# DylanAuty/ObjCAViT

Measured on AMD Instinct MI355X. Metric: images/sec (640x480, bs=16) forward depth inference, 3 batches of 16 in flight per GPU; AbsRel vs CPU ref, higher is better.
Workload: dtype f32 (fp16 / bf16 split contractions)

## Files before the change

### include/objcavit_hip.h

```cpp
#ifndef OBJCAVIT_HIP_H
#define OBJCAVIT_HIP_H

#include <stddef.h>
#include <stdint.h>

#ifdef __cplusplus
extern "C" {
#endif

typedef void* ocv_stream_t;

#define OCV_ABI_VERSION 5
int ocv_abi_version(void);
const char* ocv_last_error(void);

int ocv_range_flag_set(unsigned* flag);
int ocv_range_flag_take_fwd(unsigned* flag, unsigned* out, ocv_stream_t stream);
int ocv_attention_set_fp32_range(int on);
int ocv_attention_set_dispatch(int form);

#define OCV_ACT_NONE 0
#define OCV_ACT_RELU 1
#define OCV_ACT_LEAKY_RELU 2
#define OCV_ACT_SILU 3
// ... 126 lines not shown
int ocv_pointwise_conv_nhwc_split_fwd(const float* x, const float* gate, int rows_per_image, const void* w_packed,
                                      const float* bias, const float* residual, float* y, long M, int Cin, int Cout,
                                      int act, ocv_stream_t stream);
int ocv_pointwise_conv_nhwc_split_hl_fwd(const float* x, const float* gate, int rows_per_image, const void* w_packed,
                                         const float* bias, const float* residual, float* y, void* y_hl, long M, int Cin,
                                         int Cout, int act, ocv_stream_t stream);
size_t ocv_pointwise_split_workspace_bytes(long M, int Cin, int Cout);
int ocv_pointwise_conv_nhwc_split_ws_fwd(const float* x, const float* gate, int rows_per_image, const void* w_packed,
                                         const float* bias, const float* residual, float* y, void* y_hl, long M, int Cin, int Cout,
                                         int act, void* workspace, size_t workspace_bytes, ocv_stream_t stream);
int ocv_pointwise_hl_set_dispatch(int rt, int tn);
int ocv_pointwise_hl_fwd(const void* x_hl, int Cin, const void* w_packed, long w_image_elems, int rows_per_image,
                         const float* bias, const float* residual, float* y, void* y_hl, long M, int Cout, int act,
                         ocv_stream_t stream);
int ocv_stem_conv_fwd(const float* x, const float* w, const float* bias, float* y, int B, int Cin, int H, int W, int Cout,
                      int k, int stride, int pad_t, int pad_l, int Ho, int Wo, int act, ocv_stream_t stream);
int ocv_depthwise_conv_nhwc_fwd(const float* in, const float* w, const float* bias, float* out, int B, int C, int H,
                                int W, int k, int stride, int pad_t, int pad_l, int Ho, int Wo, int act,
                                ocv_stream_t stream);
int ocv_depthwise_set_dispatch(int mode);
int ocv_depthwise_sum_tiles(int B, int C, int Ho, int Wo, int k, int stride);
int ocv_depthwise_conv_nhwc_sum_fwd(const float* in, const float* w, const float* bias, float* out, float* part, int B,
                                    int C, int H, int W, int k, int stride, int pad_t, int pad_l, int Ho, int Wo,
                                    ocv_stream_t stream);
int ocv_se_gate_partials_fwd(const float* part, int tiles, long pixels_per_image, const float* w1, const float* b1,
                             const float* w2t, const float* b2, float* gate, float* hidden_ws, int B, int C, int R,
                             ocv_stream_t stream);
int ocv_depthwise_conv_nhwc_sum_hl_fwd(const float* in, const float* w, const float* bias, float* out, void* out_hl, float* part,
                                       int B, int C, int H, int W, int k, int stride, int pad_t, int pad_l, int Ho, int Wo,
                                       ocv_stream_t stream);
int ocv_se_gate_weights_fwd(const float* part, int tiles, long pixels_per_image, const float* w1, const float* b1,
                            const float* w2t, const float* b2, const float* W, void* w_packed, long w_image_elems, float* gate,
                            float* hidden_ws, int B, int C, int R, int N, ocv_stream_t stream);


size_t ocv_channel_mean_workspace_bytes(int B, int C, long P);
int ocv_channel_mean_nhwc_fwd(const float* x, float* out, int B, int C, long P, void* workspace, size_t workspace_bytes,
                              ocv_stream_t stream);

int ocv_se_gate_fwd(const float* mean, const float* w1, const float* b1, const float* w2t, const float* b2, float* gate,
                    float* hidden_ws, int B, int C, int R, ocv_stream_t stream);

int ocv_conv_nhwc_fwd(const float* x1, int C1, const float* x2, int C2, const void* w_hi, const void* w_lo,
                      const float* bias, const float* residual, float* y, int B, int H, int W, int Cout, int ksize,
                      int act, ocv_stream_t stream);
int ocv_conv_nhwc_exact_fwd(const float* x1, int C1, const float* x2, int C2, const float* w_tap_major, const float* bias,
                            const float* residual, float* y, int B, int H, int W, int Cout, int ksize, int act,
                            ocv_stream_t stream);
int ocv_conv3x3_nhwc_strided_fwd(const float* x, int Cin, const void* w_hi, const void* w_lo, const float* bias,
                                 const float* residual, float* y, int B, int H, int W, int Cout, int stride, int pad_t,
                                 int pad_l, int Ho, int Wo, int act, ocv_stream_t stream);

int ocv_mbconv_expand_dw_tiles(int Ho, int Wo, int k, int stride);
int ocv_mbconv_expand_dw_fwd(const float* x, const void* w_packed, const float* bias_expand, const float* w_dw,
                             const float* bias_dw, float* y, float* part, int B, int H, int W, int Cin, int mid, int k,
                             int stride, int pad_t, int pad_l, int Ho, int Wo, ocv_stream_t stream);

size_t ocv_split_act_elems(int B, int H, int W, int C);

int ocv_conv_nhwc_split_fwd(const void* x_hl, int Cin, const void* w_hi, const void* w_lo, const float* bias,
                            const float* residual, float* y, void* y_hl, int B, int H, int W, int Cout, int ksize,
                            int act, ocv_stream_t stream);
size_t ocv_conv_nhwc_split_workspace_bytes(int B, int H, int W, int Cin, int Cout, int ksize);
int ocv_conv_nhwc_split_ws_fwd(const void* x_hl, int Cin, const void* w_hi, const void* w_lo, const float* bias,
                               const float* residual, float* y, void* y_hl, int B, int H, int W, int Cout, int ksize,
                               int act, void* workspace, size_t workspace_bytes, ocv_stream_t stream);
int ocv_conv_nhwc_split_x_fwd(const void* x_hl, int Cin, const void* w_hi, const void* w_lo, const float* oscale, int f16,
                              const float* bias, const float* residual, float* y, void* y_hl, int B, int H, int W, int Cout,
                              int ksize, int act, void* workspace, size_t workspace_bytes, ocv_stream_t stream);

int ocv_conv3x3_packed_taps_k(int Cin);
int ocv_conv3x3_halo_supported(int B, int H, int W, int Cin, int Cout);
size_t ocv_conv3x3_halo_lds_bytes(void);
int ocv_conv3x3_set_dispatch(int mode);
int ocv_conv3x3_last_kernel(void);
int ocv_conv3x3_split_packed_taps_fwd(const void* x_hl, int Cin, const void* w_hi, const void* w_lo, const float* oscale, int f16,
                                      const float* bias, const float* residual, float* y, void* y_hl, int B, int H, int W, int Cout,
                                      int act, ocv_stream_t stream);

size_t ocv_conv3x3_winograd43_workspace_bytes(int B, int H, int W, int Cin, int Cout);
int ocv_conv3x3_winograd43_split_fwd(const void* x_hl, int Cin, const void* u_hi, const void* u_lo, const float* fscale,
                                     const float* cscale, const float* bias, float* y, void* y_hl, int B, int H, int W, int Cout,
                                     int act, int hl_f16, void* workspace, size_t workspace_bytes, ocv_stream_t stream);

int ocv_tap_interp_supported(int h, int w, int H, int W, int Cout);
int ocv_tap_interp_staging_rounds(int h, int w, int H, int W);
int ocv_tap_interp_combine_fwd(const float* z, int h, int w, int zpad, const float* zborder, const float* s, const float* bias,
                               float* y, void* y_hl, int B, int H, int W, int Cout, int act, ocv_stream_t stream);
int ocv_tap_interp_combine_x_fwd(const float* z, int h, int w, int zpad, const float* zborder, const float* s, const float* bias,
                                 float* y, void* y_hl, int hl_f16, int B, int H, int W, int Cout, int act, ocv_stream_t stream);


int ocv_upsample_concat_split_fwd(const float* x, int h, int w, int C1, const float* skip, int C2, void* out_hl, int B,
                                  int H, int W, ocv_stream_t stream);
int ocv_upsample_concat_split_x_fwd(const float* x, int h, int w, int C1, const float* skip, int C2, void* out_hl, int f16, int B,
                                    int H, int W, ocv_stream_t stream);

size_t ocv_depth_metrics_workspace_bytes(int B, int H, int W);
int ocv_depth_metrics_fwd(const float* pred, const float* pred_mirror, int h, int w, const float* gt, int H, int W,
                          float min_depth, float max_depth, int crop_y0, int crop_y1, int crop_x0, int crop_x1,
                          long first_image_id, float* records, int B, void* workspace, size_t workspace_bytes,
                          ocv_stream_t stream);
size_t ocv_depth_metrics_loss_workspace_bytes(int B, int H, int W, int n_bins);
int ocv_depth_metrics_loss_fwd(const float* pred, const float* pred_mirror, int h, int w, const float* gt, int H, int W,
                               float min_depth, float max_depth, int crop_y0, int crop_y1, int crop_x0, int crop_x1,
                               const float* bin_edges, int n_bins, long first_image_id, float* records, float* loss_records, int B,
// ... 65 lines not shown
```

### objcavit_amd/_lib.py

```python
from __future__ import annotations

import ctypes as C
import os
from typing import Optional

_HERE = os.path.dirname(os.path.abspath(__file__))
LIB_PATH = os.environ.get("OCV_LIB_PATH") or os.path.join(_HERE, "lib", "libobjcavit_hip.so")

_f32p = C.c_void_p
_u8p = C.c_void_p
_stream = C.c_void_p
ABI_VERSION = 5


class EncoderLayerParams(C.Structure):
    _fields_ = [("struct_size", C.c_size_t)] + [(n, C.c_void_p) for n in (
        "in_proj_w", "in_proj_b", "out_proj_w", "out_proj_b", "norm1_w", "norm1_b",
        "linear1_w", "linear1_b", "linear2_w", "linear2_b", "norm2_w", "norm2_b",
        "in_proj_p3", "out_proj_p3", "linear1_p3", "linear2_p3",
        "in_proj_h2", "out_proj_h2", "linear1_h2", "linear2_h2")]

    def __init__(self, *a, **kw):
        super().__init__(*a, **kw)
        self.struct_size = C.sizeof(EncoderLayerParams)
# ... 71 lines not shown
    "ocv_bin_head_partials_bytes": (C.c_size_t, [C.c_int, C.c_int]),
    "ocv_bin_head_folded_ws_fwd": (C.c_int, [_f32p, C.c_int, _f32p, _f32p, _f32p, _f32p, C.c_int, C.c_int, C.c_int, C.c_int,
                                             C.c_void_p, C.c_size_t, _stream]),
    "ocv_bin_head_stats_partials_bytes": (C.c_size_t, [C.c_int, C.c_int]),
    "ocv_bin_head_folded_stats_fwd": (C.c_int, [_f32p, C.c_int, _f32p, _f32p, _f32p, _f32p, C.c_int, C.c_int, C.c_int, C.c_int,
                                                C.c_void_p, C.c_size_t, _f32p, _f32p, _stream]),
    "ocv_bin_head_fwd": (C.c_int, [_f32p, C.c_int, _f32p, C.c_long, C.c_int, _f32p, _f32p, _f32p, _f32p, C.c_int, C.c_int,
                                   C.c_int, C.c_int, C.c_int, C.c_void_p, C.c_size_t, _stream]),
    "ocv_depthwise_conv_fwd": (C.c_int, [_f32p, _f32p, _f32p, _f32p] + [C.c_int] * 11 + [_stream]),
    "ocv_depthwise_set_dispatch": (C.c_int, [C.c_int]),
    "ocv_depthwise_sum_tiles": (C.c_int, [C.c_int] * 6),
    "ocv_depthwise_conv_nhwc_sum_fwd": (C.c_int, [_f32p] * 5 + [C.c_int] * 10 + [_stream]),
    "ocv_se_gate_partials_fwd": (C.c_int, [_f32p, C.c_int, C.c_long, _f32p, _f32p, _f32p, _f32p, _f32p, _f32p, C.c_int,
                                           C.c_int, C.c_int, _stream]),
    "ocv_depth_metrics_workspace_bytes": (C.c_size_t, [C.c_int] * 3),
    "ocv_depth_metrics_fwd": (C.c_int, [_f32p, _f32p, C.c_int, C.c_int, _f32p, C.c_int, C.c_int, C.c_float, C.c_float] + [C.c_int] * 4 +
                              [C.c_long, _f32p, C.c_int, C.c_void_p, C.c_size_t, _stream]),
    "ocv_depth_metrics_loss_workspace_bytes": (C.c_size_t, [C.c_int] * 4),
    "ocv_depth_metrics_loss_fwd": (C.c_int, [_f32p, _f32p, C.c_int, C.c_int, _f32p, C.c_int, C.c_int, C.c_float, C.c_float] + [C.c_int] * 4 +
                                   [_f32p, C.c_int, C.c_long, _f32p, _f32p, C.c_int, C.c_void_p, C.c_size_t, _stream]),
    "ocv_frame_ingest_fwd": (C.c_int, [_u8p, C.c_long, C.c_long, C.c_int, C.c_int, C.c_int, C.c_int, _f32p, _f32p, C.c_int, C.c_int, C.c_int,
                                       C.c_int, C.c_long, _stream]),
    "ocv_depth_ingest_fwd": (C.c_int, [C.c_void_p, C.c_long, C.c_long, C.c_int, C.c_int, C.c_int, C.c_int, C.c_float, _f32p, C.c_int, C.c_int,
                                       C.c_int, _stream]),
    "ocv_depth_finalize_fwd": (C.c_int, [_f32p, _f32p, C.c_int, C.c_int, C.c_float, C.c_float, C.c_int, C.c_int, _f32p, C.c_void_p, C.c_float,
                                         _u8p, _u8p, C.c_float, C.c_float, C.c_int, _stream]),
    "ocv_depth_finalize_stats_fwd": (C.c_int, [_f32p] * 6 + [C.c_int, C.c_int, C.c_float, C.c_float, C.c_int, C.c_int, _f32p, _f32p, C.c_int,
                                               _stream]),
    "ocv_object_depth_fwd": (C.c_int, [_f32p, _f32p, _f32p, C.c_long, C.c_void_p, C.c_int, C.c_int, C.c_int, C.c_int, C.c_float,
                                       C.POINTER(C.c_double), C.c_int, _f32p, _stream]),
    "ocv_object_metrics_workspace_bytes": (C.c_size_t, [C.c_int] * 3),
    "ocv_object_metrics_fwd": (C.c_int, [_f32p, _f32p, C.c_int, C.c_int, _f32p, C.c_int, C.c_int, C.c_float, C.c_float] + [C.c_int] * 4 +
                               [_f32p, C.c_long, C.c_void_p, C.c_int, C.c_int, C.c_float, _f32p, _f32p, C.c_void_p, C.c_size_t, _stream]),
    "ocv_depth_unproject_workspace_bytes": (C.c_size_t, [C.c_int] * 5),
    "ocv_depth_unproject_fwd": (C.c_int, [_f32p, _f32p, _f32p, _f32p, _u8p, C.c_long, C.c_long] + [C.c_int] * 9 + [C.c_float] * 4 +
                                [C.c_int, _f32p, C.c_void_p, C.c_void_p, C.c_void_p, C.c_void_p, C.c_size_t, _stream]),
    "ocv_conv3x3_few_channels_fwd": (C.c_int, [_f32p, C.c_long, C.c_long, C.c_long, C.c_long, _f32p, _f32p] + [C.c_int] * 5 + [_stream]),
    "ocv_stem_conv_fwd": (C.c_int, [_f32p, _f32p, _f32p, _f32p] + [C.c_int] * 12 + [_stream]),
    "ocv_pointwise_packed_weight_elems": (C.c_size_t, [C.c_int, C.c_int]),
    "ocv_pointwise_split_set_dispatch": (C.c_int, [C.c_int, C.c_int, C.c_int]),
    "ocv_pointwise_conv_nhwc_split_fwd": (C.c_int, [_f32p, _f32p, C.c_int, C.c_void_p, _f32p, _f32p, _f32p,
                                                    C.c_long, C.c_int, C.c_int, C.c_int, C.c_void_p]),
    "ocv_pointwise_conv_nhwc_fwd": (C.c_int, [_f32p, _f32p, C.c_int, _f32p, _f32p, _f32p, _f32p, C.c_long, C.c_int, C.c_int,
                                              C.c_int, _stream]),
    "ocv_depthwise_conv_nhwc_fwd": (C.c_int, [_f32p, _f32p, _f32p, _f32p] + [C.c_int] * 11 + [_stream]),
    "ocv_channel_mean_workspace_bytes": (C.c_size_t, [C.c_int, C.c_int, C.c_long]),
    "ocv_channel_mean_nhwc_fwd": (C.c_int, [_f32p, _f32p, C.c_int, C.c_int, C.c_long, C.c_void_p, C.c_size_t, _stream]),
    "ocv_se_gate_fwd": (C.c_int, [_f32p] * 7 + [C.c_int] * 3 + [_stream]),
    "ocv_conv_nhwc_fwd": (C.c_int, [_f32p, C.c_int, _f32p, C.c_int, C.c_void_p, C.c_void_p, _f32p, _f32p, _f32p] +
                          [C.c_int] * 6 + [_stream]),
    "ocv_conv3x3_nhwc_strided_fwd": (C.c_int, [_f32p, C.c_int, C.c_void_p, C.c_void_p, _f32p, _f32p, _f32p] + [C.c_int] * 10 + [_stream]),
    "ocv_conv_nhwc_exact_fwd": (C.c_int, [_f32p, C.c_int, _f32p, C.c_int, _f32p, _f32p, _f32p, _f32p] + [C.c_int] * 6 + [_stream]),
    "ocv_mbconv_expand_dw_tiles": (C.c_int, [C.c_int] * 4),
    "ocv_mbconv_expand_dw_fwd": (C.c_int, [_f32p, C.c_void_p, _f32p, _f32p, _f32p, _f32p, _f32p] + [C.c_int] * 11 + [_stream]),
    "ocv_regressor_bins_fwd": (C.c_int, [_f32p, C.c_long, _f32p, _f32p, _f32p, _f32p, _f32p, _f32p, C.c_int, C.c_int, C.c_int, C.c_int, C.c_float,
                                         C.c_int, C.c_float, C.c_float, _f32p, _f32p, _f32p, C.c_int, _stream]),
    "ocv_bin_edges_fwd": (C.c_int, [_f32p, C.c_int, C.c_float, C.c_float, _f32p, _f32p, _f32p, C.c_int, C.c_int, _stream]),
    "ocv_object_tokens_pad_fwd": (C.c_int, [_f32p, C.c_void_p, C.c_float, _f32p, _u8p, C.c_int, C.c_int, C.c_int, _stream]),
    "ocv_object_front_pad_fwd": (C.c_int, [_f32p, C.c_void_p, C.c_int, C.c_int, C.c_float, _f32p, _u8p] + [C.c_int] * 4 + [_stream]),
    "ocv_object_frontend_fwd": (C.c_int, [_f32p, C.c_long, C.c_void_p, C.c_void_p, C.c_int, C.c_int, C.c_void_p, C.c_int, C.c_void_p, C.c_void_p,
                                          C.c_int, C.c_void_p, C.c_int, C.POINTER(C.c_float), C.c_int, C.c_int, C.c_float, _f32p, C.c_long,
                                          C.c_long, _f32p, C.c_long, C.c_long, C.c_void_p, C.c_int, C.c_void_p, C.c_void_p, _u8p, _stream]),
    "ocv_split_act_elems": (C.c_size_t, [C.c_int] * 4),
    "ocv_conv_nhwc_split_fwd": (C.c_int, [C.c_void_p, C.c_int, C.c_void_p, C.c_void_p, _f32p, _f32p, _f32p, C.c_void_p]
                                + [C.c_int] * 6 + [_stream]),
    "ocv_conv_nhwc_split_workspace_bytes": (C.c_size_t, [C.c_int] * 6),
    "ocv_conv_nhwc_split_ws_fwd": (C.c_int, [C.c_void_p, C.c_int, C.c_void_p, C.c_void_p, _f32p, _f32p, _f32p, C.c_void_p]
                                   + [C.c_int] * 6 + [C.c_void_p, C.c_size_t, _stream]),
    "ocv_conv_nhwc_split_x_fwd": (C.c_int, [C.c_void_p, C.c_int, C.c_void_p, C.c_void_p, _f32p, C.c_int, _f32p, _f32p, _f32p, C.c_void_p]
                                  + [C.c_int] * 6 + [C.c_void_p, C.c_size_t, _stream]),
    "ocv_conv3x3_packed_taps_k": (C.c_int, [C.c_int]),
    "ocv_conv3x3_halo_supported": (C.c_int, [C.c_int] * 5),
    "ocv_conv3x3_halo_lds_bytes": (C.c_size_t, []),
    "ocv_conv3x3_set_dispatch": (C.c_int, [C.c_int]),
    "ocv_conv3x3_last_kernel": (C.c_int, []),
    "ocv_conv3x3_split_packed_taps_fwd": (C.c_int, [C.c_void_p, C.c_int, C.c_void_p, C.c_void_p, _f32p, C.c_int, _f32p, _f32p, _f32p, C.c_void_p]
                                          + [C.c_int] * 5 + [_stream]),
    "ocv_upsample_concat_split_x_fwd": (C.c_int, [_f32p, C.c_int, C.c_int, C.c_int, _f32p, C.c_int, C.c_void_p, C.c_int,
                                                  C.c_int, C.c_int, C.c_int, _stream]),
    "ocv_tap_interp_combine_x_fwd": (C.c_int, [_f32p, C.c_int, C.c_int, C.c_int, _f32p, _f32p, _f32p, _f32p, C.c_void_p] + [C.c_int] * 6 + [_stream]),
    "ocv_pos_grid_sample_fwd": (C.c_int, [_f32p, C.c_int, C.c_int, C.c_int, _f32p, C.c_int, C.c_int, C.c_int, C.c_float, C.c_float,
                                          C.c_int, _f32p, _f32p, _stream]),
    "ocv_conv3x3_winograd43_workspace_bytes": (C.c_size_t, [C.c_int] * 5),
    "ocv_conv3x3_winograd43_split_fwd": (C.c_int, [C.c_void_p, C.c_int, C.c_void_p, C.c_void_p, _f32p, _f32p, _f32p, _f32p, C.c_void_p] + [C.c_int] * 6 +
                                         [C.c_void_p, C.c_size_t, _stream]),
    "ocv_tap_interp_supported": (C.c_int, [C.c_int] * 5),
    "ocv_tap_interp_staging_rounds": (C.c_int, [C.c_int] * 4),
    "ocv_tap_interp_combine_fwd": (C.c_int, [_f32p, C.c_int, C.c_int, C.c_int, _f32p, _f32p, _f32p, _f32p, C.c_void_p] + [C.c_int] * 5 + [_stream]),
    "ocv_upsample_concat_split_fwd": (C.c_int, [_f32p, C.c_int, C.c_int, C.c_int, _f32p, C.c_int, C.c_void_p,
                                                C.c_int, C.c_int, C.c_int, _stream]),
}

_lib: Optional[C.CDLL] = None


class HipLibraryError(RuntimeError):
    pass


def load(path: Optional[str] = None) -> C.CDLL:
    global _lib
    if _lib is not None and path is None:
        return _lib
    import torch
    p = path or LIB_PATH
    if not os.path.exists(p):
# ... 26 lines not shown
```

### objcavit_amd/csrc/mbconv_fused.hip

```cpp
#include "common.hpp"
#include "../../include/objcavit_hip.h"

namespace {

typedef __bf16 bf16x8 __attribute__((ext_vector_type(8)));

struct FXArgs {
  const float *x, *be, *wd, *bd;
  const __bf16* wp;
  float *y, *part;
  int Cin, mid, H, W, Ho, Wo, pad_t, pad_l;
  int tiles_x, tiles_per_image, nchunks;
};

template <int K, int S>
struct FXGeom {
  static constexpr int TH = 8, TW = S == 1 ? 32 : 16;
  static constexpr int RG = 256 / (8 * TW);
  static constexpr int NR = TH / RG;
  static constexpr int IH = (TH - 1) * S + K, IW = (TW - 1) * S + K;
  static constexpr int P = IH * IW, MT = (P + 31) / 32;
  static constexpr int HALF = (IW + 1) / 2;
  static constexpr int NLI = (NR - 1) * S + K;
  static constexpr int LDS_BYTES = MT * 32 * 32 * 4;
// ... 135 lines not shown
      const int d = li - ky;
      if (d >= 0 && d % S == 0 && d / S < G::NR) {
#pragma unroll
        for (int kx = 0; kx < K; ++kx) acc[d / S] = fx_fma4(wdw[ky * K + kx], v[kx], acc[d / S]);
      }
    }
  }
  float4 psum = make_float4(0.f, 0.f, 0.f, 0.f);
  const int ox = ox0 + col;
  float* orow = p.y + (((long)b * p.Ho + oy0 + rg * G::NR) * p.Wo + ox) * p.mid + cq;
  const long ostep = (long)p.Wo * p.mid;
#pragma unroll
  for (int o = 0; o < G::NR; ++o, orow += ostep) {
    const int oy = oy0 + rg * G::NR + o;
    if (cok && oy < p.Ho && ox < p.Wo) {
      float4 r = acc[o];
      r.x = fast_silu(r.x); r.y = fast_silu(r.y); r.z = fast_silu(r.z); r.w = fast_silu(r.w);
      *reinterpret_cast<float4*>(orow) = r;
      psum.x += r.x; psum.y += r.y; psum.z += r.z; psum.w += r.w;
    }
  }
  __syncthreads();
  *reinterpret_cast<float4*>(e + (tid >> 3) * 32 + 4 * q) = psum;
  __syncthreads();
  if (tid < 32 && n0 + tid < p.mid) {
    float s = 0.f;
#pragma unroll 8
    for (int j = 0; j < 32; ++j) s += e[j * 32 + tid];
    p.part[((long)b * p.tiles_per_image + t2) * p.mid + n0 + tid] = s;
  }
}

template <int K, int S, int KS>
int fx_launch(const FXArgs& a, int B, hipStream_t st) {
  using G = FXGeom<K, S>;
  static bool attr = false;
  if (!attr) {
    (void)hipFuncSetAttribute((const void*)mbconv_expand_dw_kernel<K, S, KS>, hipFuncAttributeMaxDynamicSharedMemorySize, G::LDS_BYTES);
    attr = true;
  }
  const long grid = (long)B * a.tiles_per_image * a.nchunks;
  hipLaunchKernelGGL((mbconv_expand_dw_kernel<K, S, KS>), dim3((unsigned)grid), dim3(256), G::LDS_BYTES, st, a);
  OCV_CHECK_LAUNCH("ocv_mbconv_expand_dw_fwd");
  return 0;
}

template <int K, int S>
int fx_dispatch_ks(const FXArgs& a, int B, int ks, hipStream_t st) {
  if (ks == 2) return fx_launch<K, S, 2>(a, B, st);
  if (ks == 3) return fx_launch<K, S, 3>(a, B, st);
  return fx_launch<K, S, 4>(a, B, st);
}

}

extern "C" int ocv_mbconv_expand_dw_tiles(int Ho, int Wo, int k, int stride) {
  if (Ho < 1 || Wo < 1 || (k != 3 && k != 5) || (stride != 1 && stride != 2)) return 0;
  const int tw = stride == 1 ? 32 : 16;
  return ((Ho + 7) / 8) * ((Wo + tw - 1) / tw);
}

namespace {
int fx_run(const float* x, const void* w_packed, const float* bias_expand, const float* w_dw, const float* bias_dw, float* y,
           float* part, int B, int H, int W, int Cin, int mid, int k, int stride, int pad_t, int pad_l,
           int Ho, int Wo, ocv_stream_t stream) {
  OCV_CHECK_ARG(x && w_packed && w_dw && y && part, "ocv_mbconv_expand_dw_fwd: null pointer");
  OCV_CHECK_ARG(B >= 1 && H >= 1 && W >= 1 && Ho >= 1 && Wo >= 1, "ocv_mbconv_expand_dw_fwd: bad sizes");
  OCV_CHECK_ARG(Cin >= 24 && Cin % 8 == 0 && Cin <= 64, "ocv_mbconv_expand_dw_fwd: Cin must be a multiple of 8 in [24, 64] (got %d)", Cin);
  OCV_CHECK_ARG(mid >= 4 && mid % 4 == 0, "ocv_mbconv_expand_dw_fwd: expanded channels must be a multiple of 4 (got %d)", mid);
  OCV_CHECK_ARG((k == 3 || k == 5) && (stride == 1 || stride == 2), "ocv_mbconv_expand_dw_fwd: k must be 3 or 5 and stride 1 or 2 (got k=%d s=%d)", k, stride);
  OCV_CHECK_ARG(pad_t >= 0 && pad_l >= 0 && pad_t < k && pad_l < k, "ocv_mbconv_expand_dw_fwd: bad padding");
  OCV_CHECK_ARG((Ho - 1) * stride - pad_t < H && (Wo - 1) * stride - pad_l < W, "ocv_mbconv_expand_dw_fwd: output larger than the padded input allows");
  OCV_CHECK_ARG(ocv_aligned16(x) && ocv_aligned16(w_packed) && ocv_aligned16(w_dw) && ocv_aligned16(bias_dw) && ocv_aligned16(y),
                "ocv_mbconv_expand_dw_fwd: operands must be 16-byte aligned");
  FXArgs a{};
  a.x = x; a.be = bias_expand; a.wd = w_dw; a.bd = bias_dw; a.wp = (const __bf16*)w_packed; a.y = y; a.part = part;
  a.Cin = Cin; a.mid = mid; a.H = H; a.W = W; a.Ho = Ho; a.Wo = Wo; a.pad_t = pad_t; a.pad_l = pad_l;
  const int tw = stride == 1 ? 32 : 16;
  a.tiles_x = (Wo + tw - 1) / tw;
  a.tiles_per_image = ((Ho + 7) / 8) * a.tiles_x;
  a.nchunks = (mid + 31) / 32;
  OCV_CHECK_ARG((long)B * a.tiles_per_image * a.nchunks < (1L << 31), "ocv_mbconv_expand_dw_fwd: too many work items");
  const int ks = (Cin + 15) / 16;
  hipStream_t st = (hipStream_t)stream;
  if (k == 3 && stride == 1) return fx_dispatch_ks<3, 1>(a, B, ks, st);
  if (k == 3 && stride == 2) return fx_dispatch_ks<3, 2>(a, B, ks, st);
  if (k == 5 && stride == 1) return fx_dispatch_ks<5, 1>(a, B, ks, st);
  return fx_dispatch_ks<5, 2>(a, B, ks, st);
}
}

extern "C" int ocv_mbconv_expand_dw_fwd(const float* x, const void* w_packed, const float* bias_expand, const float* w_dw,
                                        const float* bias_dw, float* y, float* part, int B, int H, int W, int Cin, int mid,
                                        int k, int stride, int pad_t, int pad_l, int Ho, int Wo, ocv_stream_t stream) {
  return fx_run(x, w_packed, bias_expand, w_dw, bias_dw, y, part, B, H, W, Cin, mid, k, stride, pad_t, pad_l, Ho, Wo, stream);
}
```

### objcavit_amd/hip_ops/encoder.py

```python
from __future__ import annotations

import ctypes as C
import math
import os
import threading
from typing import Dict, Optional, Sequence, Tuple

import torch

from .. import _lib
from .._lib import EncoderLayerParams, check
from ._core import *
from .conv import *


def depthwise_conv_same(x: torch.Tensor, weight: torch.Tensor, bias: Optional[torch.Tensor], stride: int,
                        act: int = ACT_NONE) -> torch.Tensor:
    lib = _lib.load()
    _req(x, "x"); _req(weight, "weight")
    B, Cc, H, W = x.shape
    k = weight.shape[-1]
    if weight.shape != (Cc, 1, k, k):
        raise ValueError(f"depthwise_conv_same: weight {tuple(weight.shape)} does not match {Cc} channels")
    if bias is not None:
# ... 311 lines not shown
            _req(t, n)
    R = w1.shape[0]
    N = w_proj.shape[0]
    if w1.shape != (R, Cc) or w2t.shape != (R, Cc) or b1.numel() != R or b2.numel() != Cc or tuple(w_proj.shape) != (N, Cc):
        raise ValueError("depthwise_se_gate_weights: parameter shape mismatch")
    Ho, Wo, pt, pl = _out_pad(H, W, k, stride, padding)
    tiles = lib.ocv_depthwise_sum_tiles(B, Cc, Ho, Wo, k, stride)
    if tiles <= 0:
        raise ValueError("depthwise_se_gate_weights: unsupported shape")
    ys = SplitAct.empty(B, Cc, Ho, Wo, x.device)
    part = workspace(B * tiles * Cc * 4, x.device, "dw_part")
    hid = workspace(B * R * 4, x.device, "se_hidden")
    img_elems = int(lib.ocv_pointwise_packed_weight_elems(Cc, N))
    wpk = torch.empty(B * img_elems, dtype=torch.bfloat16, device=x.device)
    gate = torch.empty(B, Cc, dtype=torch.float32, device=x.device) if want_gate else None
    with timed(f"depthwise|{B},{H},{W},{Cc},k{k}s{stride}"):
        check(lib.ocv_depthwise_conv_nhwc_sum_hl_fwd(x.data_ptr(), weight_kkc.data_ptr(), _ptr(bias), None, ys.hl.data_ptr(),
                                                     part.data_ptr(), B, Cc, H, W, k, stride, pt, pl, Ho, Wo,
                                                     _stream()), "ocv_depthwise_conv_nhwc_sum_hl_fwd")
    with timed("se_gate_weights"):
        check(lib.ocv_se_gate_weights_fwd(part.data_ptr(), tiles, Ho * Wo, w1.data_ptr(), b1.data_ptr(), w2t.data_ptr(),
                                          b2.data_ptr(), w_proj.data_ptr(), wpk.data_ptr(), img_elems, _ptr(gate), hid.data_ptr(),
                                          B, Cc, R, N, _stream()), "ocv_se_gate_weights_fwd")
    wg = PerImageSplitWeight(wpk, N, Cc, img_elems, B)
    return (ys, wg, gate) if want_gate else (ys, wg)


def expand_depthwise_fusable(cin: int, weight, k: int = 3) -> bool:
    return isinstance(weight, SplitWeight) and 24 <= cin <= 64 and cin % 8 == 0 and k == 3


def expand_depthwise_se_gate(x: torch.Tensor, w_expand: "SplitWeight", b_expand: Optional[torch.Tensor], weight_kkc: torch.Tensor,
                             bias: Optional[torch.Tensor], k: int, stride: int, w1: torch.Tensor, b1: torch.Tensor,
                             w2t: torch.Tensor, b2: torch.Tensor, padding: Optional[Tuple[int, int]] = None):
    lib = _lib.load()
    x = _nhwc(x, "x")
    B, Cin, H, W = x.shape
    if not isinstance(w_expand, SplitWeight) or w_expand.cin != Cin:
        raise ValueError("expand_depthwise_se_gate: expand weight must be a SplitWeight matching x's channels")
    _req(w_expand.packed, "w_expand.packed", torch.bfloat16)
    mid = w_expand.cout
    _req(weight_kkc, "weight")
    if weight_kkc.shape != (k * k, mid):
        raise ValueError(f"expand_depthwise_se_gate: depthwise weight {tuple(weight_kkc.shape)} does not match k={k}, C={mid}")
    for n, t in (("b_expand", b_expand), ("bias", bias), ("w1", w1), ("b1", b1), ("w2t", w2t), ("b2", b2)):
        if t is not None:
            _req(t, n)
    R = w1.shape[0]
    if w1.shape != (R, mid) or w2t.shape != (R, mid) or b1.numel() != R or b2.numel() != mid:
        raise ValueError("expand_depthwise_se_gate: squeeze-excite parameter shape mismatch")
    if (b_expand is not None and b_expand.numel() != mid) or (bias is not None and bias.numel() != mid):
        raise ValueError("expand_depthwise_se_gate: bias size mismatch")
    Ho, Wo, pt, pl = _out_pad(H, W, k, stride, padding)
    tiles = lib.ocv_mbconv_expand_dw_tiles(Ho, Wo, k, stride)
    if tiles <= 0:
        raise ValueError("expand_depthwise_se_gate: unsupported shape")
    out = torch.empty(B, mid, Ho, Wo, dtype=torch.float32, device=x.device, memory_format=torch.channels_last)
    part = workspace(B * tiles * mid * 4, x.device, "dw_part")
    gate = torch.empty(B, mid, dtype=torch.float32, device=x.device)
    hid = workspace(B * R * 4, x.device, "se_hidden")
    with timed(f"expand_dw|{B},{H},{W},{Cin},{mid},k{k}s{stride}"):
        check(lib.ocv_mbconv_expand_dw_fwd(x.data_ptr(), w_expand.packed.data_ptr(), _ptr(b_expand), weight_kkc.data_ptr(),
                                           _ptr(bias), out.data_ptr(), part.data_ptr(), B, H, W, Cin, mid, k, stride,
                                           pt, pl, Ho, Wo, _stream()), "ocv_mbconv_expand_dw_fwd")
    with timed("se_gate"):
        check(lib.ocv_se_gate_partials_fwd(part.data_ptr(), tiles, Ho * Wo, w1.data_ptr(), b1.data_ptr(), w2t.data_ptr(),
                                           b2.data_ptr(), gate.data_ptr(), hid.data_ptr(), B, mid, R, _stream()),
              "ocv_se_gate_partials_fwd")
    return out, gate


def channel_mean_nhwc(x: torch.Tensor) -> torch.Tensor:
    lib = _lib.load()
    x = _nhwc(x, "x")
    B, Cc, H, W = x.shape
    nb = lib.ocv_channel_mean_workspace_bytes(B, Cc, H * W)
    if nb == 0:
        raise ValueError("channel_mean_nhwc: unsupported shape")
    ws = workspace(nb, x.device, "mean")
    out = torch.empty(B, Cc, dtype=torch.float32, device=x.device)
    check(lib.ocv_channel_mean_nhwc_fwd(x.data_ptr(), out.data_ptr(), B, Cc, H * W, ws.data_ptr(), ws.numel(), _stream()),
          "ocv_channel_mean_nhwc_fwd")
    return out


def se_gate(x: torch.Tensor, w1: torch.Tensor, b1: torch.Tensor, w2t: torch.Tensor, b2: torch.Tensor) -> torch.Tensor:
    lib = _lib.load()
    m = channel_mean_nhwc(x)
    B, Cc = m.shape
    for n, t in (("w1", w1), ("b1", b1), ("w2t", w2t), ("b2", b2)):
        _req(t, n)
    R = w1.shape[0]
    if w1.shape != (R, Cc) or w2t.shape != (R, Cc) or b1.numel() != R or b2.numel() != Cc:
        raise ValueError("se_gate: parameter shape mismatch")
    gate = torch.empty_like(m)
    hid = workspace(B * R * 4, x.device, "se_hidden")
    check(lib.ocv_se_gate_fwd(m.data_ptr(), w1.data_ptr(), b1.data_ptr(), w2t.data_ptr(), b2.data_ptr(), gate.data_ptr(),
                              hid.data_ptr(), B, Cc, R, _stream()), "ocv_se_gate_fwd")
    return gate


__all__ = [_n for _n in dir() if not _n.startswith("__")]
```

Before: 1138.

## Add row-ring fused expand+depthwise MBConv kernel for large stride-1 3x3 layers

Adds a new fused MBConv kernel for stride-1 3x3 layers. It streams input rows through a four-row LDS ring. Each wave computes the bf16-split expand GEMM for one row with MFMA while the depthwise 3x3 and SiLU run on earlier rows. Each workgroup covers 128 channels, a 30-column strip and a band of rows chosen by a simple cost model. It writes the squeeze-excite pooling partials per tile. Automatic dispatch sends only large activations to the new path. The aim is to cut the halo recompute and weight reloads of the old 8x32 tile kernel and to raise MFMA use. The trade-offs are serialisation inside each band, a per-row barrier, and a dispatch check that tests a fixed Cin instead of the real input channel count.

```diff
diff --git a/include/objcavit_hip.h b/include/objcavit_hip.h
--- a/include/objcavit_hip.h
+++ b/include/objcavit_hip.h
@@ -202,6 +202,10 @@
                                  int pad_l, int Ho, int Wo, int act, ocv_stream_t stream);
 
 int ocv_mbconv_expand_dw_tiles(int Ho, int Wo, int k, int stride);
+int ocv_mbconv_expand_dw_tiles_for(int B, int mid, int Ho, int Wo, int k, int stride);
+int ocv_mbconv_set_dispatch(int mode);
+int ocv_mbconv_rows_supported(int Cin, int mid, int k, int stride);
+int ocv_mbconv_rows_geometry(int B, int mid, int Ho, int Wo, int* geom5);
 int ocv_mbconv_expand_dw_fwd(const float* x, const void* w_packed, const float* bias_expand, const float* w_dw,
                              const float* bias_dw, float* y, float* part, int B, int H, int W, int Cin, int mid, int k,
                              int stride, int pad_t, int pad_l, int Ho, int Wo, ocv_stream_t stream);
diff --git a/objcavit_amd/_lib.py b/objcavit_amd/_lib.py
--- a/objcavit_amd/_lib.py
+++ b/objcavit_amd/_lib.py
@@ -147,6 +147,10 @@
     "ocv_conv3x3_nhwc_strided_fwd": (C.c_int, [_f32p, C.c_int, C.c_void_p, C.c_void_p, _f32p, _f32p, _f32p] + [C.c_int] * 10 + [_stream]),
     "ocv_conv_nhwc_exact_fwd": (C.c_int, [_f32p, C.c_int, _f32p, C.c_int, _f32p, _f32p, _f32p, _f32p] + [C.c_int] * 6 + [_stream]),
     "ocv_mbconv_expand_dw_tiles": (C.c_int, [C.c_int] * 4),
+    "ocv_mbconv_expand_dw_tiles_for": (C.c_int, [C.c_int] * 6),
+    "ocv_mbconv_set_dispatch": (C.c_int, [C.c_int]),
+    "ocv_mbconv_rows_supported": (C.c_int, [C.c_int] * 4),
+    "ocv_mbconv_rows_geometry": (C.c_int, [C.c_int] * 4 + [C.POINTER(C.c_int)]),
     "ocv_mbconv_expand_dw_fwd": (C.c_int, [_f32p, C.c_void_p, _f32p, _f32p, _f32p, _f32p, _f32p] + [C.c_int] * 11 + [_stream]),
     "ocv_regressor_bins_fwd": (C.c_int, [_f32p, C.c_long, _f32p, _f32p, _f32p, _f32p, _f32p, _f32p, C.c_int, C.c_int, C.c_int, C.c_int, C.c_float,
                                          C.c_int, C.c_float, C.c_float, _f32p, _f32p, _f32p, C.c_int, _stream]),
diff --git a/objcavit_amd/csrc/mbconv_fused.hip b/objcavit_amd/csrc/mbconv_fused.hip
--- a/objcavit_amd/csrc/mbconv_fused.hip
+++ b/objcavit_amd/csrc/mbconv_fused.hip
@@ -211,12 +211,293 @@
   return fx_launch<K, S, 4>(a, B, st);
 }
 
-}
-
-extern "C" int ocv_mbconv_expand_dw_tiles(int Ho, int Wo, int k, int stride) {
+struct MRArgs {
+  const float *x, *be, *wd, *bd;
+  const __bf16* wp;
+  float *y, *part;
+  int Cin, mid, H, W, Ho, Wo, pad_t, pad_l;
+  int nxt, TH, tiles, chunks;
+};
+
+struct MRShape {
+  static constexpr int NT = 4, CH = 32 * NT, CQ = CH / 4;
+  static constexpr int THREADS = 64 * NT;
+  static constexpr int PX = 4, NG = THREADS / CQ;
+  static constexpr int RW = 32, TW = RW - 2;
+  static constexpr int PIX = CH + 8;
+  static constexpr int NB = 4, ROWF = (RW + 2) * PIX;
+  static constexpr size_t LDS = (size_t)NB * ROWF * sizeof(float);
+  static_assert(PX * NG >= TW && PX * (NG - 1) < TW && THREADS * 4 <= NB * ROWF, "column groups cover the strip; the pooling sums reuse the ring");
+  static_assert(2 * LDS <= 160 * 1024, "two workgroups per CU");
+};
+
+typedef float f32x2 __attribute__((ext_vector_type(2)));
+__device__ __forceinline__ f32x2 fast_silu2(f32x2 x) {
+  const f32x2 t = x * -1.44269504088896340736f;
+  const f32x2 e = {__builtin_amdgcn_exp2f(t.x), __builtin_amdgcn_exp2f(t.y)};
+  const f32x2 d = 1.0f + e;
+  const f32x2 s = {__builtin_amdgcn_rcpf(d.x), __builtin_amdgcn_rcpf(d.y)};
+  return x * s;
+}
+
+template <int S, int KS>
+__global__ __launch_bounds__(MRShape::THREADS, 2) void mbconv_rows_kernel(MRArgs p) {
+  static_assert(S == 1, "stride 2 stays on mbconv_expand_dw_kernel");
+  using G = MRShape;
+  constexpr int PIX = G::PIX, NB = G::NB, ROWF = G::ROWF, PX = G::PX;
+  extern __shared__ __attribute__((aligned(16))) float mr_ring[];
+  const int tid = threadIdx.x, lane = tid & 63, l31 = lane & 31, hh = lane >> 5;
+  const int wave = __builtin_amdgcn_readfirstlane(tid >> 6);
+  int tile, chunk;
+  long b;
+  {
+    const int nwg = gridDim.x;
+    int wg = blockIdx.x;
+    const int qq = nwg >> 3, r = nwg & 7, xcd = wg & 7, idx = wg >> 3;
+    wg = (xcd < r ? xcd * (qq + 1) : r * (qq + 1) + (xcd - r) * qq) + idx;
+    chunk = wg % p.chunks;
+    const int rest = wg / p.chunks;
+    tile = rest % p.tiles;
+    b = rest / p.tiles;
+  }
+  const int band = tile / p.nxt, xt = tile - band * p.nxt;
+  const int y0 = band * p.TH, nout = min(p.Ho, y0 + p.TH) - y0;
+  const int iyb = y0 - p.pad_t, ixb = xt * G::TW - p.pad_l;
+  const int n0 = chunk * G::CH;
+  const int nrel = nout + 2;
+
+  const int c0 = n0 + 32 * wave;
+  bf16x8 bh[KS], bl[KS];
+  {
+    const int ct = c0 < p.mid ? c0 >> 5 : 0;
+#pragma unroll
+    for (int s = 0; s < KS; ++s) {
+      const __bf16* f = p.wp + (((long)ct * KS + s) * 2) * 512 + lane * 8;
+      bh[s] = *reinterpret_cast<const bf16x8*>(f);
+      bl[s] = *reinterpret_cast<const bf16x8*>(f + 512);
+    }
+  }
+  const bool nok = c0 + l31 < p.mid;
+  const float bev = (nok && p.be != nullptr) ? p.be[c0 + l31] : 0.f;
+  unsigned msk = 0;
+#pragma unroll
+  for (int r = 0; r < 16; ++r) msk |= nok && (unsigned)(ixb + acc_row(r, hh)) < (unsigned)p.W ? 1u << r : 0u;
+  const bool colsin = ixb >= 0 && ixb + G::RW <= p.W && c0 + 32 <= p.mid;
+  const float* xb = p.x + b * (long)p.H * p.W * p.Cin;
+  const int ixc = min(max(ixb + l31, 0), p.W - 1);
+  int koff[KS];
+#pragma unroll
+  for (int s = 0; s < KS; ++s) koff[s] = ixc * p.Cin + min(16 * s + 8 * hh, p.Cin - 8);
+  float4 raw[KS][2];
+  auto loadrow = [&](int rel) {
+    const int iy = min(max(iyb + min(rel, nrel - 1), 0), p.H - 1);
+    const float* row = xb + (long)iy * p.W * p.Cin;
+#pragma unroll
+    for (int s = 0; s < KS; ++s) {
+      raw[s][0] = ld4(row + koff[s]);
+      raw[s][1] = ld4(row + koff[s] + 4);
+    }
+  };
+  auto expand = [&](int next) -> f32x16 {
+    bf16x8 ah[KS], al[KS];
+#pragma unroll
+    for (int s = 0; s < KS; ++s) fx_split8(raw[s][0], raw[s][1], ah[s], al[s]);
+    loadrow(next);
+    f32x16 acc;
+#pragma unroll
+    for (int r = 0; r < 16; ++r) acc[r] = bev;
+#pragma unroll
+    for (int s = 0; s < KS; ++s) {
+      acc = __builtin_amdgcn_mfma_f32_32x32x16_bf16(ah[s], bh[s], acc, 0, 0, 0);
+      acc = __builtin_amdgcn_mfma_f32_32x32x16_bf16(ah[s], bl[s], acc, 0, 0, 0);
+      acc = __builtin_amdgcn_mfma_f32_32x32x16_bf16(al[s], bh[s], acc, 0, 0, 0);
+    }
+    return acc;
+  };
+  float* const wbase = mr_ring + 4 * hh * PIX + 32 * wave + l31;
+  auto put = [&](const f32x16& acc, int rel) {
+    float* dst = wbase + (rel & (NB - 1)) * ROWF;
+    if (colsin && (unsigned)(iyb + rel) < (unsigned)p.H) {
+#pragma unroll
+      for (int r = 0; r < 16; r += 2) {
+        const f32x2 v = fast_silu2(f32x2{acc[r], acc[r + 1]});
+        dst[acc_row(r, 0) * PIX] = v.x;
+        dst[acc_row(r + 1, 0) * PIX] = v.y;
+      }
+    } else {
+      const unsigned m = (unsigned)(iyb + rel) < (unsigned)p.H ? msk : 0u;
+#pragma unroll
+      for (int r = 0; r < 16; r += 2) {
+        const f32x2 v = fast_silu2(f32x2{acc[r], acc[r + 1]});
+        dst[acc_row(r, 0) * PIX] = (m >> r) & 1u ? v.x : 0.f;
+        dst[acc_row(r + 1, 0) * PIX] = (m >> (r + 1)) & 1u ? v.y : 0.f;
+      }
+    }
+  };
+
+  const int q = tid & (G::CQ - 1), g = tid / G::CQ;
+  const int cq = n0 + 4 * q;
+  const bool cok = cq < p.mid;
+  const int ox = xt * G::TW + g * PX;
+  const int nval = cok ? max(min(min(G::TW - g * PX, p.Wo - ox), PX), 0) : 0;
+  const int cqs = cok ? cq : 0;
+  float4 wdw[9];
+#pragma unroll
+  for (int t = 0; t < 9; ++t) wdw[t] = ld4(p.wd + (unsigned)(t * p.mid + cqs));
+  const float4 bdw = p.bd != nullptr ? ld4(p.bd + cqs) : make_float4(0.f, 0.f, 0.f, 0.f);
+  const float* const rbase = mr_ring + g * PX * PIX + 4 * q;
+  unsigned voff[PX];
+#pragma unroll
+  for (int o = 0; o < PX; ++o) voff[o] = o < nval ? (unsigned)(((ox + o) * p.mid + cq) * 4) : 0x80000000u;
+  const float* orow = p.y + (b * p.Ho + y0) * (long)p.Wo * p.mid;
+  const long ostep = (long)p.Wo * p.mid;
+  const int rowbytes = p.Wo * p.mid * 4;
+  f32x2 ps[PX][2];
+#pragma unroll
+  for (int o = 0; o < PX; ++o) ps[o][0] = ps[o][1] = f32x2{0.f, 0.f};
+  auto depthwise = [&](int n) {
+    float4 acc[PX];
+#pragma unroll
+    for (int o = 0; o < PX; ++o) acc[o] = bdw;
+#pragma unroll
+    for (int ky = 0; ky < 3; ++ky) {
+      const float* rr = rbase + ((n + ky) & (NB - 1)) * ROWF;
+      float4 v[PX + 2];
+#pragma unroll
+      for (int j = 0; j < PX + 2; ++j) v[j] = *reinterpret_cast<const float4*>(rr + j * PIX);
+#pragma unroll
+      for (int kx = 0; kx < 3; ++kx)
+#pragma unroll
+        for (int o = 0; o < PX; ++o) acc[o] = fx_fma4(wdw[ky * 3 + kx], v[o + kx], acc[o]);
+    }
+    const __amdgpu_buffer_rsrc_t rs = __builtin_amdgcn_make_buffer_rsrc(const_cast<float*>(orow), 0, rowbytes, 0x00020000);
+#pragma unroll
+    for (int o = 0; o < PX; ++o) {
+      const f32x2 lo = fast_silu2(f32x2{acc[o].x, acc[o].y}), hi = fast_silu2(f32x2{acc[o].z, acc[o].w});
+      __builtin_amdgcn_raw_buffer_store_b128(f32x4{lo.x, lo.y, hi.x, hi.y}, rs, voff[o], 0, 0);
+      ps[o][0] += lo;
+      ps[o][1] += hi;
+    }
+    orow += ostep;
+  };
+
+  loadrow(0);
+#pragma unroll 1
+  for (int rel = 0; rel < 3; ++rel) {
+    const f32x16 acc = expand(rel + 1);
+    put(acc, rel);
+  }
+#pragma unroll 1
+  for (int n = 0; n < nout - 1; ++n) {
+    asm volatile("s_waitcnt lgkmcnt(0)" ::: "memory");
+    __builtin_amdgcn_s_barrier();
+    asm volatile("" ::: "memory");
+    const f32x16 acc = expand(n + 4);
+    depthwise(n);
+    put(acc, n + 3);
+  }
+  asm volatile("s_waitcnt lgkmcnt(0)" ::: "memory");
+  __builtin_amdgcn_s_barrier();
+  asm volatile("" ::: "memory");
+  depthwise(nout - 1);
+
+  __syncthreads();
+  float4 psum = make_float4(0.f, 0.f, 0.f, 0.f);
+#pragma unroll
+  for (int o = 0; o < PX; ++o)
+    if (o < nval) { psum.x += ps[o][0].x; psum.y += ps[o][0].y; psum.z += ps[o][1].x; psum.w += ps[o][1].y; }
+  float4* red = reinterpret_cast<float4*>(mr_ring);
+  red[tid] = psum;
+  __syncthreads();
+  if (tid < G::CQ && n0 + 4 * tid < p.mid) {
+    float4 t = red[tid];
+#pragma unroll
+    for (int gg = 1; gg < G::NG; ++gg) {
+      const float4 u = red[gg * G::CQ + tid];
+      t.x += u.x; t.y += u.y; t.z += u.z; t.w += u.w;
+    }
+    float* dst = p.part + (b * p.tiles + tile) * (long)p.mid + n0 + 4 * tid;
+    dst[0] = t.x; dst[1] = t.y; dst[2] = t.z; dst[3] = t.w;
+  }
+}
+
+struct MRGeom { int chunks, nxt, TH, tiles; };
+MRGeom mr_geom(int B, int mid, int Ho, int Wo) {
+  MRGeom g{};
+  g.chunks = (mid + MRShape::CH - 1) / MRShape::CH;
+  g.nxt = (Wo + MRShape::TW - 1) / MRShape::TW;
+  long best = -1;
+  for (int nb = 1; nb <= Ho; ++nb) {
+    const int th = (Ho + nb - 1) / nb;
+    if (nb > 1 && th < 8) break;
+    const long wgs = (long)B * g.chunks * g.nxt * ((Ho + th - 1) / th);
+    const long cost = ((wgs + 511) / 512) * (th + 2);
+    if (best < 0 || cost < best) {
+      best = cost;
+      g.TH = th;
+    }
+  }
+  g.tiles = g.nxt * ((Ho + g.TH - 1) / g.TH);
+  return g;
+}
+
+int& mr_dispatch() {
+  static int mode = 0;
+  return mode;
+}
+bool mr_supported(int Cin, int mid, int k, int stride) {
+  return Cin >= 24 && Cin <= 64 && Cin % 8 == 0 && mid >= 4 && mid % 4 == 0 && k == 3 && stride == 1;
+}
+bool mr_use_rows(int B, int mid, int Ho, int Wo, int k, int stride) {
+  const int mode = mr_dispatch();
+  if (mode == 1 || !mr_supported(24, mid, k, stride)) return false;
+  const MRGeom g = mr_geom(B, mid, Ho, Wo);
+  if ((long)B * g.chunks * g.tiles >= (1L << 31)) return false;
+  if (((long)Wo + 4) * 64 >= (1L << 30) || (long)Wo * mid * 4 >= (1L << 31)) return false;
+  return mode == 2 || (long)B * Ho * Wo * mid >= 16L * 120 * 160 * 240;
+}
+
+template <int KS>
+int mr_launch(const MRArgs& a, int B, hipStream_t st) {
+  static bool attr = false;
+  if (!attr) {
+    (void)hipFuncSetAttribute((const void*)mbconv_rows_kernel<1, KS>, hipFuncAttributeMaxDynamicSharedMemorySize, (int)MRShape::LDS);
+    attr = true;
+  }
+  const long grid = (long)B * a.chunks * a.tiles;
+  hipLaunchKernelGGL((mbconv_rows_kernel<1, KS>), dim3((unsigned)grid), dim3(MRShape::THREADS), MRShape::LDS, st, a);
+  OCV_CHECK_LAUNCH("ocv_mbconv_expand_dw_fwd");
+  return 0;
+}
+
+int fx_tiles(int Ho, int Wo, int k, int stride) {
   if (Ho < 1 || Wo < 1 || (k != 3 && k != 5) || (stride != 1 && stride != 2)) return 0;
   const int tw = stride == 1 ? 32 : 16;
   return ((Ho + 7) / 8) * ((Wo + tw - 1) / tw);
+}
+
+}
+
+extern "C" int ocv_mbconv_expand_dw_tiles(int Ho, int Wo, int k, int stride) { return fx_tiles(Ho, Wo, k, stride); }
+
+extern "C" int ocv_mbconv_set_dispatch(int mode) {
+  OCV_CHECK_ARG(mode >= 0 && mode <= 2, "ocv_mbconv_set_dispatch: mode must be 0 (automatic), 1 (tile kernel) or 2 (row ring), got %d", mode);
+  mr_dispatch() = mode;
+  return 0;
+}
+
+extern "C" int ocv_mbconv_rows_supported(int Cin, int mid, int k, int stride) { return mr_supported(Cin, mid, k, stride) ? 1 : 0; }
+
+extern "C" int ocv_mbconv_rows_geometry(int B, int mid, int Ho, int Wo, int* geom5) {
+  OCV_CHECK_ARG(geom5 != nullptr && B >= 1 && Ho >= 1 && Wo >= 1 && mid >= 4 && mid % 4 == 0, "ocv_mbconv_rows_geometry: bad arguments");
+  const MRGeom g = mr_geom(B, mid, Ho, Wo);
+  geom5[0] = g.chunks; geom5[1] = MRShape::CH; geom5[2] = g.nxt; geom5[3] = MRShape::TW; geom5[4] = g.TH;
+  return 0;
+}
+
+extern "C" int ocv_mbconv_expand_dw_tiles_for(int B, int mid, int Ho, int Wo, int k, int stride) {
+  if (B < 1 || mid < 4 || mid % 4 != 0 || fx_tiles(Ho, Wo, k, stride) == 0) return 0;
+  return mr_use_rows(B, mid, Ho, Wo, k, stride) ? mr_geom(B, mid, Ho, Wo).tiles : fx_tiles(Ho, Wo, k, stride);
 }
 
 namespace {
@@ -234,14 +515,25 @@
                 "ocv_mbconv_expand_dw_fwd: operands must be 16-byte aligned");
   FXArgs a{};
   a.x = x; a.be = bias_expand; a.wd = w_dw; a.bd = bias_dw; a.wp = (const __bf16*)w_packed; a.y = y; a.part = part;
+  const int ks = (Cin + 15) / 16;
+  hipStream_t st = (hipStream_t)stream;
+  if (mr_use_rows(B, mid, Ho, Wo, k, stride)) {
+    OCV_CHECK_ARG((long)W * Cin < (1L << 31), "ocv_mbconv_expand_dw_fwd: input row too large");
+    MRArgs r{};
+    r.x = x; r.be = bias_expand; r.wd = w_dw; r.bd = bias_dw; r.wp = (const __bf16*)w_packed; r.y = y; r.part = part;
+    r.Cin = Cin; r.mid = mid; r.H = H; r.W = W; r.Ho = Ho; r.Wo = Wo; r.pad_t = pad_t; r.pad_l = pad_l;
+    const MRGeom g = mr_geom(B, mid, Ho, Wo);
+    r.nxt = g.nxt; r.TH = g.TH; r.tiles = g.tiles; r.chunks = g.chunks;
+    if (ks == 2) return mr_launch<2>(r, B, st);
+    if (ks == 3) return mr_launch<3>(r, B, st);
+    return mr_launch<4>(r, B, st);
+  }
   a.Cin = Cin; a.mid = mid; a.H = H; a.W = W; a.Ho = Ho; a.Wo = Wo; a.pad_t = pad_t; a.pad_l = pad_l;
   const int tw = stride == 1 ? 32 : 16;
   a.tiles_x = (Wo + tw - 1) / tw;
   a.tiles_per_image = ((Ho + 7) / 8) * a.tiles_x;
   a.nchunks = (mid + 31) / 32;
   OCV_CHECK_ARG((long)B * a.tiles_per_image * a.nchunks < (1L << 31), "ocv_mbconv_expand_dw_fwd: too many work items");
-  const int ks = (Cin + 15) / 16;
-  hipStream_t st = (hipStream_t)stream;
   if (k == 3 && stride == 1) return fx_dispatch_ks<3, 1>(a, B, ks, st);
   if (k == 3 && stride == 2) return fx_dispatch_ks<3, 2>(a, B, ks, st);
   if (k == 5 && stride == 1) return fx_dispatch_ks<5, 1>(a, B, ks, st);
diff --git a/objcavit_amd/hip_ops/encoder.py b/objcavit_amd/hip_ops/encoder.py
--- a/objcavit_amd/hip_ops/encoder.py
+++ b/objcavit_amd/hip_ops/encoder.py
@@ -387,7 +387,7 @@
     if (b_expand is not None and b_expand.numel() != mid) or (bias is not None and bias.numel() != mid):
         raise ValueError("expand_depthwise_se_gate: bias size mismatch")
     Ho, Wo, pt, pl = _out_pad(H, W, k, stride, padding)
-    tiles = lib.ocv_mbconv_expand_dw_tiles(Ho, Wo, k, stride)
+    tiles = lib.ocv_mbconv_expand_dw_tiles_for(B, mid, Ho, Wo, k, stride)
     if tiles <= 0:
         raise ValueError("expand_depthwise_se_gate: unsupported shape")
     out = torch.empty(B, mid, Ho, Wo, dtype=torch.float32, device=x.device, memory_format=torch.channels_last)
```

Result: no change. 1149, median of 6 (+1.0%).
